# hyperplane-lab/RGBManip

Hardware: AMD Instinct MI355X
Metric: adapose_poses_per_sec_batch256 (higher is better)
Workload: dtype bf16

## Files before the change

### rgbmanip_amd/_lib.py

```python
from __future__ import annotations

import ctypes as C
import os

_HERE = os.path.dirname(os.path.abspath(__file__))
LIB_PATH = os.environ.get("RGBM_HIP_LIB") or os.path.join(_HERE, "librgbm_hip.so")

F32, BF16, F16, BF16X3 = 0, 1, 2, 3
ACT_NONE, ACT_RELU, ACT_PRELU, ACT_TANH = 0, 1, 2, 3
RES_NONE, RES_PRE_ACT, RES_POST_ACT = 0, 1, 2


PROF_ROWS = 42
PROF_KERNELS = [
    ("conv_igemm_glds_kernel<float, 16, 256>", "fp32"), ("conv_igemm_glds_kernel<float, 32, 256>", "fp32"),
    ("conv_igemm_glds_kernel<float, 64, 256>", "fp32"), ("conv_igemm_glds_kernel<float, 128, 128>", "fp32"),
    ("conv_igemm_glds_kernel<unsigned short, 16, 256>", "bf16"), ("conv_igemm_glds_kernel<unsigned short, 32, 256>", "bf16"),
    ("conv_igemm_glds_kernel<unsigned short, 64, 256>", "bf16"), ("conv_igemm_glds_kernel<unsigned short, 128, 128>", "bf16"),
    ("conv3d_tile_kernel<float, ...> (conv1..conv11)", "fp32"), ("conv3d_tile_kernel<unsigned short, ...> (conv1..conv11)", "bf16"),
    ("conv3d_tile_kernel<float, 32, 16, 4, 8, 8, 1, false, true> (conv0 + fused plane sweep)", "fp32"),
    ("conv3d_tile_kernel<unsigned short, 32, 16, 4, 8, 8, 1, false, true> (conv0 + fused plane sweep)", "bf16"),
    ("conv_igemm_ws_kernel<float, ...>", "fp32"), ("conv_igemm_ws_kernel<unsigned short, false, false> (128 channels x 256 pixels)", "bf16"),
    ("conv0_sweep_persistent_kernel<unsigned short> (conv0 + fused plane sweep of bf16 nets; sweep_f16 = 0 / fp16 nets: conv0_sweep_kernel)", "bf16"), ("conv_igemm_ws64_kernel", "bf16"),
    ("conv3d_tile_kernel<unsigned short, 32, 16, 6, 8, 8, 1, false, false> (conv0 on a materialised volume)", "bf16"),
    ("conv3d_tile_kernel<unsigned short, 8, 16, 2, 8, 8, 2, false, false> (conv1)", "bf16"),
    ("conv3d_tile_kernel<unsigned short, 16, 16, 4, 8, 8, 1, false, false> (conv2)", "bf16"),
    ("conv3d_tile_kernel<unsigned short, 16, 32, 2, 8, 8, 2, false, false> (conv3)", "bf16"),
    ("conv3d_tile_kernel<unsigned short, 32, 32, 2, 8, 8, 1, false, false> (conv4)", "bf16"),
    ("conv3d_tile_kernel<unsigned short, 32, 64, 1, 8, 8, 2, false, false> (conv5)", "bf16"),
    ("conv3d_tile_kernel<unsigned short, 64, 64, 1, 8, 8, 1, false, false> (conv6)", "bf16"),
    ("conv3d_tile_kernel<unsigned short, 64, 32, 1, 8, 8, 1, true, false> (conv7)", "bf16"),
    ("conv3d_tile_kernel<unsigned short, 32, 16, 2, 8, 8, 1, true, false> (conv9)", "bf16"),
    ("conv3d_tile_kernel<unsigned short, 16, 16, 4, 8, 8, 1, true, false> (conv11)", "bf16"),
] + [("conv_igemm_glds_kernel<bx3_t, ...> (all channel tiles)", "bf16x3"), ("conv3d_tile_kernel<bx3_t, ...> (conv1..conv11)", "bf16x3"),
     ("conv0 + fused plane sweep <bx3_t>", "bf16x3"), ("conv_igemm_ws_kernel<rgbm::bx3_t, false, false> (128 channels x 256 pixels)", "bf16x3"),
     ("unused (conv_igemm_w256_kernel of rounds 2-5)", "bf16"),
     ("conv_igemm_m32_kernel<unsigned short, 256, 256> (256 channels x 256 pixels, 32x32x16 MFMAs; gemm_kernel = 0: conv_igemm_ws_kernel<unsigned short, true, false>, 256 x 128)", "bf16"),
     ("unused (row-halo ws tile of rounds 2-5)", "bf16"),
     ("conv_igemm_m32_kernel<rgbm::bx3_t, 256, 256> (256 channels x 256 pixels, 32x32x16 MFMAs; gemm_kernel = 0: conv_igemm_ws_kernel<rgbm::bx3_t, true, false>, 256 x 128)", "bf16x3"),
     ("conv_igemm_ws_kernel<rgbm::bx3_t, false, false, true> (64 channels x 256 pixels, four multiply waves)", "bf16x3"),
     ("conv_igemm_ws_kernel<unsigned short, false, false, true> (64 channels x 256 pixels, four multiply waves)", "bf16"),
     ("conv_igemm_ws_kernel<float, false, false, true> (64 channels x 256 pixels, four multiply waves)", "fp32"),
     ("upconv_combine_kernel<16-bit> (PSPUpsample tap combination)", "bf16"), ("upconv_combine_kernel<4-byte> (PSPUpsample tap combination)", "bf16x3"),
     ("upconv_final_kernel (up_3 + final in one kernel; either storage width)", "bf16"),
     ("conv_igemm_m32_kernel<unsigned short, 128, 64 / 128 / 256> (128-pixel tiles: tail and small-batch launches of the 256-channel GEMM)", "bf16"),
     ("conv_igemm_m32_kernel<rgbm::bx3_t, 128, 64 / 128 / 256> (128-pixel tiles: tail and small-batch launches of the 256-channel GEMM)", "bf16x3")]
assert len(PROF_KERNELS) == PROF_ROWS


class RgbmError(RuntimeError):
    pass


class WeightDesc(C.Structure):
    _fields_ = [("name", C.c_char_p), ("data", C.c_void_p), ("ndim", C.c_int), ("shape", C.POINTER(C.c_int64))]


class PolicyLayout(C.Structure):
    _fields_ = [("dims", C.c_int * 5), ("log_std", C.c_int), ("w", (C.c_int * 4) * 2), ("b", (C.c_int * 4) * 2), ("total", C.c_int)]


POLICY_MAX_HIDDEN, POLICY_MAX_WIDTH, POLICY_MAX_ACT = 6, 512, 32
POLICY_ACTIVATIONS = {"elu": 0, "selu": 1, "relu": 2, "crelu": 2, "lrelu": 3, "tanh": 4, "sigmoid": 5}


class PolicyDesc(C.Structure):
    _fields_ = [("obs_dim", C.c_int), ("state_dim", C.c_int), ("act_dim", C.c_int), ("activation", C.c_int), ("asymmetric", C.c_int),
                ("n_hidden", C.c_int * 2), ("hidden", (C.c_int * POLICY_MAX_HIDDEN) * 2),
                ("w", (C.c_int * (POLICY_MAX_HIDDEN + 1)) * 2), ("b", (C.c_int * (POLICY_MAX_HIDDEN + 1)) * 2),
                ("log_std", C.c_int), ("total", C.c_int)]


class AdaposeOut(C.Structure):
    _fields_ = [(n, C.c_void_p) for n in ("view1_nocs", "view2_nocs", "view1_depth", "view2_depth", "view1_r", "view2_r",
                                           "view1_t", "view2_t", "view1_s", "view2_s")]


class ControlRewardArgs(C.Structure):
    _fields_ = [(n, C.c_void_p) for n in ("action", "cam_pose", "target", "move_success", "bbox", "avail", "gt_bbox", "pred_bbox",
                                           "pose_cur", "pose_prev", "robot_pose", "success", "reward", "terms")] + [
        ("coef", C.c_double * 14), ("proper_pos", C.c_double * 3), ("precision2", C.c_double),
        ("N", C.c_int), ("T", C.c_int), ("lda", C.c_int), ("pots", C.c_int), ("first", C.c_int), ("pad_", C.c_int)]


class SynthScene(C.Structure):
    _fields_ = [("cam_pose", C.c_void_p), ("robot_pose", C.c_void_p), ("box", C.c_void_p),
                ("fx", C.c_double), ("fy", C.c_double), ("cx", C.c_double), ("cy", C.c_double),
                ("N", C.c_int), ("H", C.c_int), ("W", C.c_int), ("env0", C.c_int)]


_vp, _i, _f, _d, _sz, _i64 = C.c_void_p, C.c_int, C.c_float, C.c_double, C.c_size_t, C.c_int64
# ... 112 lines not shown
```

### rgbmanip_amd/csrc/adapose.cpp

```cpp
#include "adapose.h"

#include <math.h>
#include <string.h>

namespace rgbm {

static const int kLayerPlanes[4] = {64, 128, 256, 512};
static const int kLayerBlocks[4] = {3, 4, 6, 3};
static const int kLayerStride[4] = {1, 2, 1, 1};
static const int kLayerDil[4] = {1, 1, 2, 4};
static const int kPspBins[4] = {1, 2, 3, 6};
static const int kPspSmallViews = 32;


static const HostTensor* find(const StateDict& sd, const std::string& name) {
  auto it = sd.find(name);
  return it == sd.end() ? nullptr : &it->second;
}

#define GET(var, name)                                               \
  const HostTensor* var = find(sd, name);                            \
  RGBM_REQUIRE(var != nullptr, std::string("missing weight ") + (name))

static int init_conv2d(ConvLayer& L, int dtype, const StateDict& sd, const std::string& wname, const char* bname, int Cin,
// ... 564 lines not shown
  const size_t VP = (size_t)V * P;

  if (int rc = launch_stage_in(P1, P2, choose1, choose2, bf.Pviews, bf.choose, B, P, s)) return rc;
  const float* drop = nullptr;
  if (drop_active()) {
    RGBM_REQUIRE(V <= drop_cap_views && drop_masks && (drop_explicit || drop_state), "dropout: mask buffer smaller than the batch");
    RGBM_REQUIRE((upconv & 3) == 3, "dropout needs option upconv bits 0 and 1 (up_1 / up_2 through the tap combination)");
    if (drop_explicit) {
      RGBM_REQUIRE(drop_explicit == B, "dropout: the masks set for the next forward are for batch " + std::to_string(drop_explicit));
      drop_explicit = 0;
    } else {
      if (int rc = launch_dropout_masks(drop_masks, drop_state, B, drop_p, drop_seed, drop_no_advance ? 0 : 1, s)) return rc;
    }
    drop = drop_masks;
    drop_last_B = B;
  }
  if (int rc = pspnet(bf, V, img1, img2, s, drop)) return rc;
  if (int rc = launch_homography(bf.Pviews, bf.homog, V, B, s)) return rc;
  if (dtype == BF16X3 && !feat_f32_only())
    if (int rc = launch_bx3_to_f32(bf.feat, bf.featf, (long long)V * S * S * 32, s)) return rc;
  if (stop_after == 1) return 0;
  (void)VP; (void)P; (void)D;
  return heads(bf, B, depths, out, s, stop_after);
}

int AdaPose::heads(const Buffers& bf, int B, const float* depths, const Outputs& out, hipStream_t s, int stop_after) const {
  const int V = 2 * B, P = n_pts, S = img, D = n_depth;
  const void* featg = bf.feat;
  int fdt = dtype;
  if (dtype == BF16X3) { featg = bf.featf; fdt = F32; }
  if (feat_f16()) fdt = F16;

  const int Vh = view2_heads ? V : B;
  if (pmlp_table != nullptr && !(g_debug_flags & DBG_POINT_MLP_R5) && ((long long)Vh * P) % 64 == 0) {
    PointMlpDesc pd{};
    pd.table = pmlp_table; pd.feat = featg; pd.choose = bf.choose; pd.nocs4 = bf.nocs4; pd.pf = bf.PF96 + 32; pd.ldpf = 96; pd.P = P; pd.HW = S * S;
    pd.N = (long long)Vh * P;
    if (int rc = launch_point_mlp(fdt, pd, s)) return rc;
  } else {
    if (int rc = launch_gather_points(fdt, featg, bf.choose, bf.X0, Vh, P, S * S, 32, s)) return rc;
    if (int rc = inst.run(bf.X0, bf.X1, Vh, 1, 1, P, 64, nullptr, 0, nullptr, 0, s)) return rc;
    if (int rc = nh[0].run(bf.X1, bf.H128, Vh, 1, 1, P, 128, nullptr, 0, nullptr, 0, s)) return rc;
    if (int rc = nh[1].run(bf.H128, bf.H64, Vh, 1, 1, P, 64, nullptr, 0, nullptr, 0, s)) return rc;
    if (int rc = nh[2].run(bf.H64, bf.nocs4, Vh, 1, 1, P, 4, nullptr, 0, nullptr, 0, s)) return rc;
    if (int rc = npm[0].run(bf.nocs4, bf.N32, Vh, 1, 1, P, 32, nullptr, 0, nullptr, 0, s)) return rc;
    if (int rc = npm[1].run(bf.N32, bf.PF96 + 32, Vh, 1, 1, P, 96, nullptr, 0, nullptr, 0, s)) return rc;
  }

  if (int rc = cost_volume(bf, V, B, depths, s)) return rc;
  if (stop_after == 2) return 0;

  if (int rc = launch_fuse_points(fdt, featg, bf.homog, depths, bf.choose, bf.prob, bf.PF96, V, B, P, D, S, S, 96, 0, s, Vh)) return rc;
  const int pdt = pose_dtype();
  const void* pf_in = bf.PF96;
  if (pdt == F16) {
    if (int rc = launch_f32_to_f16(bf.PF96, bf.PF96h, (long long)Vh * P * 96, s)) return rc;
    pf_in = bf.PF96h;
  } else if (pdt == BF16X3) {
    if (int rc = launch_f32_to_bx3(bf.PF96, bf.PF96, (long long)Vh * P * 96, s)) return rc;
  }
  if (int rc = pm1[0].run(pf_in, bf.Q128a, Vh, 1, 1, P, 128, nullptr, 0, nullptr, 0, s)) return rc;
  if (int rc = pm1[1].run(bf.Q128a, bf.Q128b, Vh, 1, 1, P, 128, nullptr, 0, nullptr, 0, s)) return rc;
  if (int rc = launch_mean_points_partial(pdt, bf.Q128b, (float*)bf.Q128a, Vh, P, 128, s)) return rc;
  if (int rc = launch_view_linear_mean((const float*)bf.Q128a, P, bf.glob, pm2_0_wfull, pm2_0_bias, bf.vbias, Vh, 128, 256, 256, 128, 0, s)) return rc;
  if (int rc = pm2[0].run(bf.Q128b, bf.G256a, Vh, 1, 1, P, 256, nullptr, 0, bf.vbias, 256, s)) return rc;
  if (int rc = pm2[1].run(bf.G256a, bf.G256b, Vh, 1, 1, P, 256, nullptr, 0, nullptr, 0, s)) return rc;
  if (int rc = launch_mean_points_partial(pdt, bf.G256b, (float*)bf.G256a, Vh, P, 256, s)) return rc;
  float* hout[3] = {bf.r6, bf.tv, bf.sv};
  const int hdim[3] = {6, 3, 3};
  if (int rc = launch_pose_heads_mean((const float*)bf.G256a, P, bf.pf2, bf.R, head_w, head_b, hout, hdim, Vh, s)) return rc;

  {
    float* const on[2] = {out.nocs1, out.nocs2};
    float* const od[2] = {out.depth1, out.depth2};
    float* const orr[2] = {out.r1, out.r2};
    float* const ot[2] = {out.t1, out.t2};
    float* const os[2] = {out.s1, out.s2};
    if (int rc = launch_stage_out(bf.nocs4, bf.depth, bf.R, bf.tv, bf.sv, on, od, orr, ot, os, B, P, view2_heads, s)) return rc;
  }
  return 0;
}

int AdaPose::feature_parts(const Buffers& bf, FeaturePart parts[2]) const {
  const size_t one = (size_t)img * img * 32;
  if (dtype != BF16X3) { parts[0] = {bf.feat, 0, one * dtype_size(dtype)}; return 1; }
  if (feat_f32_only()) { parts[0] = {bf.featf, 0, one * 4}; return 1; }
  parts[0] = {bf.feat, 0, one * 4};
  parts[1] = {bf.featf, one * 4, one * 4};
  return 2;
}

size_t AdaPose::feature_bytes() const {
  Buffers bf{};
  FeaturePart parts[2];
  const int n = feature_parts(bf, parts);
  return parts[n - 1].off + parts[n - 1].bytes;
}

size_t AdaPose::features_workspace_bytes(int V) const { return workspace_bytes((V + 1) / 2); }

int AdaPose::features(int V, const float* images, const int* slots, void* pool, int pool_records, void* workspace, size_t workspace_size,
                      hipStream_t s) const {
  RGBM_REQUIRE(V > 0 && pool_records > 0, "features: views and pool records");
  RGBM_REQUIRE(!drop_active(), "features: Dropout2d is on (its masks are drawn per pose and per forward, so a kept feature map would change "
               "what the net computes); the feature cache needs set_dropout(0)");
  RGBM_REQUIRE(((uintptr_t)workspace & 255) == 0 && ((uintptr_t)pool & 15) == 0, "features: workspace must be 256-byte, pool 16-byte aligned");
  const size_t need = features_workspace_bytes(V);
  RGBM_REQUIRE(workspace_size >= need, "features workspace too small: need " + std::to_string(need));
  Arena A(workspace, workspace_size);
  Buffers bf;
  plan((V + 1) / 2, A, bf);
  if (int rc = pspnet(bf, V, images, nullptr, s, nullptr)) return rc;
  if (dtype == BF16X3 && !feat_f32_only())
    if (int rc = launch_bx3_to_f32(bf.feat, bf.featf, (long long)V * img * img * 32, s)) return rc;
  FeaturePart parts[2];
  const int np = feature_parts(bf, parts);
  const size_t rec = feature_bytes();
  for (int i = 0; i < np; ++i)
    if (int rc = launch_feature_store(parts[i].buf, pool, slots, V, pool_records, parts[i].off, parts[i].bytes, rec, s)) return rc;
  return 0;
// ... 31 lines not shown
```

### rgbmanip_amd/csrc/head_kernels.hip

```cpp
#include "common.h"
#include "kernels.h"

namespace rgbm {

template <typename T>
__global__ void gather_points_kernel(const T* __restrict__ feat, const int* __restrict__ choose, float* __restrict__ out,
                                     int V, int P, int HW, int C) {
  const int q = C / 4;
  const long long total = (long long)V * P * q;
  for (long long i = blockIdx.x * (long long)blockDim.x + threadIdx.x; i < total; i += (long long)gridDim.x * blockDim.x) {
    const int c4 = (int)(i % q);
    const long long vp = i / q;
    const long long v = vp / P;
    const int pix = choose[vp];
    float x[4];
    load4(feat + (v * HW + pix) * C + c4 * 4, x);
    store4(out + vp * C + c4 * 4, x);
  }
}

int launch_gather_points(int dtype, const void* feat, const int* choose, float* out, int V, int P, int HW, int C,
                         hipStream_t s) {
  const long long total = (long long)V * P * (C / 4);
  const unsigned g = (unsigned)((total + 255) / 256);
// ... 294 lines not shown
      const bool xin0 = (unsigned)x0 < (unsigned)W, xin1 = (unsigned)(x0 + 1) < (unsigned)W;
      const bool yin0 = (unsigned)y0 < (unsigned)H, yin1 = (unsigned)(y0 + 1) < (unsigned)H;
      const int xc0 = min(max(x0, 0), W - 1), xc1 = min(max(x0 + 1, 0), W - 1);
      const int yc0 = min(max(y0, 0), H - 1), yc1 = min(max(y0 + 1, 0), H - 1);
      float s00[4], s01[4], s10[4], s11[4];
      load4(src + ((long long)yc0 * W + xc0) * C, s00);
      load4(src + ((long long)yc0 * W + xc1) * C, s01);
      load4(src + ((long long)yc1 * W + xc0) * C, s10);
      load4(src + ((long long)yc1 * W + xc1) * C, s11);
      const float w00 = (xin0 && yin0) ? (1.f - tx) * (1.f - ty) : 0.f, w01 = (xin1 && yin0) ? tx * (1.f - ty) : 0.f;
      const float w10 = (xin0 && yin1) ? (1.f - tx) * ty : 0.f, w11 = (xin1 && yin1) ? tx * ty : 0.f;
      const float pr = prob[vp * D + dz];
#pragma unroll
      for (int e = 0; e < 4; ++e) {
        float wv = 0.f;
        if (xin0 && yin0) wv += s00[e] * w00;
        if (xin1 && yin0) wv += s01[e] * w01;
        if (xin0 && yin1) wv += s10[e] * w10;
        if (xin1 && yin1) wv += s11[e] * w11;
        if (!fin) wv = __builtin_nanf("");
        float f = ref[e] + wv;
        if (ROUND_BF16) f = round_through<T>(f);
        acc[e] += f * pr;
      }
    }
    store4(out + vp * ldo + ch_off + c4 * 4, acc);
  }
}

int launch_fuse_points(int dtype, const void* feat, const float* homog, const float* depths, const int* choose,
                       const float* prob, float* out, int V, int B, int P, int D, int H, int W, int ldo, int ch_off,
                       hipStream_t s, int Vn) {
  if (Vn < 0) Vn = V;
  const long long total = (long long)Vn * P * 8;
  RGBM_REQUIRE(D >= 1 && D <= 24 && total > 0 && (total + 255) / 256 < (1ll << 31), "fuse_points supports up to 24 depth planes");
  RGBM_REQUIRE((P & 7) == 0, "fuse_points: the point count must be a multiple of 8 (a wave's 8 points share one view's homography)");
  const unsigned g = (unsigned)((total + 255) / 256);
  if (dtype == BF16)
    hipLaunchKernelGGL((fuse_points_kernel<unsigned short, true>), dim3(g), dim3(256), 0, s, (const unsigned short*)feat,
                       homog, depths, choose, prob, out, V, B, P, D, H, W, ldo, ch_off, Vn);
  else if (dtype == F16)
    hipLaunchKernelGGL((fuse_points_kernel<f16_t, true>), dim3(g), dim3(256), 0, s, (const f16_t*)feat,
                       homog, depths, choose, prob, out, V, B, P, D, H, W, ldo, ch_off, Vn);
  else if (dtype == BF16X3)
    hipLaunchKernelGGL((fuse_points_kernel<bx3_t, false>), dim3(g), dim3(256), 0, s, (const bx3_t*)feat,
                       homog, depths, choose, prob, out, V, B, P, D, H, W, ldo, ch_off, Vn);
  else
    hipLaunchKernelGGL((fuse_points_kernel<float, false>), dim3(g), dim3(256), 0, s, (const float*)feat, homog, depths,
                       choose, prob, out, V, B, P, D, H, W, ldo, ch_off, Vn);
  RGBM_CHECK_HIP(hipGetLastError());
  return 0;
}

constexpr int kMeanSplit = 8;
template <typename TI>
__global__ __launch_bounds__(256) void mean_points_kernel(const TI* __restrict__ in, float* __restrict__ partial, int P, int C) {
  constexpr int E = 16 / sizeof(TI);
  __shared__ float part[256 * E];
  const int v = blockIdx.x / kMeanSplit, sl = blockIdx.x % kMeanSplit;
  const int p0 = (int)((long long)P * sl / kMeanSplit), p1 = (int)((long long)P * (sl + 1) / kMeanSplit);
  const int tpr = C / E, rows = 256 / tpr;
  const int cc = threadIdx.x % tpr, rp = threadIdx.x / tpr;
  float acc[E];
#pragma unroll
  for (int e = 0; e < E; ++e) acc[e] = 0.f;
  if (rp < rows)
#pragma unroll 8
    for (int p = p0 + rp; p < p1; p += rows) {
      float t[E];
      unpack_chunk(*reinterpret_cast<const uint4*>(in + ((long long)v * P + p) * C + cc * E), t, TI());
#pragma unroll
      for (int e = 0; e < E; ++e) acc[e] += t[e];
    }
  if (rp < rows) {
#pragma unroll
    for (int e = 0; e < E; ++e) part[rp * C + cc * E + e] = acc[e];
  }
  __syncthreads();
  for (int c = threadIdx.x; c < C; c += 256) {
    float sum = 0.f;
    for (int r = 0; r < rows; ++r) sum += part[r * C + c];
    partial[(long long)blockIdx.x * C + c] = sum;
  }
}

__device__ __forceinline__ float mean_from_partials(const float* __restrict__ partial, long long v, int c, int C, int P) {
  float sum = 0.f;
#pragma unroll
  for (int sl = 0; sl < kMeanSplit; ++sl) sum += partial[(v * kMeanSplit + sl) * C + c];
  return sum / (float)P;
}

__global__ __launch_bounds__(256) void mean_points_finish_kernel(const float* __restrict__ partial, float* __restrict__ out, int P, int C) {
  const int v = blockIdx.x;
  for (int c = threadIdx.x; c < C; c += 256) out[(long long)v * C + c] = mean_from_partials(partial, v, c, C, P);
}

int launch_mean_points_partial(int dtype, const void* in, float* scratch, int V, int P, int C, hipStream_t s) {
  RGBM_REQUIRE(dtype == F32 || dtype == F16 || dtype == BF16X3, "mean_points: fp32, fp16 or split-pair input");
  RGBM_REQUIRE(scratch != nullptr && (const void*)scratch != in, "mean_points: scratch");
  const int E = dtype == F16 ? 8 : 4;
  RGBM_REQUIRE(C % E == 0 && C / E <= 256 && 256 % (C / E) == 0, "mean_points: channel count");
  const dim3 g((unsigned)V * kMeanSplit);
  if (dtype == F16)
    hipLaunchKernelGGL(mean_points_kernel<f16_t>, g, dim3(256), 0, s, (const f16_t*)in, scratch, P, C);
  else if (dtype == BF16X3)
    hipLaunchKernelGGL(mean_points_kernel<bx3_t>, g, dim3(256), 0, s, (const bx3_t*)in, scratch, P, C);
// ... 251 lines not shown
```

### rgbmanip_amd/csrc/kernels.h

```cpp
#pragma once
#include <vector>

#include "common.h"

namespace rgbm {

int launch_nchw_to_nhwc_pad(int dtype, const float* in, void* out, int V, int C, int H, int W, int Cp, hipStream_t s);
int launch_maxpool3x3s2(int dtype, const void* in, void* out, int V, int H, int W, int C, hipStream_t s);
int launch_resize_bilinear_ac(int dtype, const void* in, void* out, int V, int Hs, int Ws, int C, int Ho, int Wo, int ldo,
                              int ch_off, hipStream_t s);
int launch_copy_channels(int dtype, const void* in, void* out, long long npix, int C, int ldo, int ch_off, hipStream_t s);
int launch_adaptive_avgpool(int dtype, const void* in, void* out, int V, int H, int W, int C, int S, hipStream_t s);
int launch_adaptive_avgpool_multi(int dtype, const void* in, void* const* outs, const int* bins, int nb, int V, int H, int W, int C,
                                  hipStream_t s);
int launch_psp_pool_conv(int dtype, const void* in, int ldi, const void* const* w, void* const* outs, const int* bins, int V, int H, int W,
                         int act, float slope, hipStream_t s);
int launch_psp_resize_cat(int dtype, const void* f, const void* const* stages, const int* bins, void* out, int V, int Ho, int Wo, hipStream_t s);
int launch_homography(const float* P_views, float* out, int V, int B, hipStream_t s);
int launch_build_volume(int dtype, const void* feat, const float* homog, const float* depths, void* vol, int v0, int Vc, int V,
                        int B, int D, int H, int W, hipStream_t s);

int launch_upconv_combine(int dtype, const void* z, const float* bias, void* out, int V, int h, int w, int Co, int ldo, int act,
                          float slope, hipStream_t s, const float* drop = nullptr);
int launch_upconv_final(int dtype, const void* x, const void* wz, const float* bias, float slope, const void* wf, const float* biasf,
                        void* out, int out_f32, int V, int h, int w, hipStream_t s, const void* wf_f16 = nullptr);

constexpr int kDropoutPerView = 256 + 64;
unsigned dropout_threshold(float p);
float dropout_scale(float p);
int launch_dropout_masks(float* masks, unsigned long long* state, int B, float p, unsigned long long seed, int advance, hipStream_t s);

size_t bn_scratch_bytes(int V);
int launch_bn_per_sample(int dtype, void* y, const void* res, const float* gamma, const float* beta, void* scratch, int V,
                         long long nvox, int C, int relu, hipStream_t s);

int launch_to_f32(int dtype, const void* in, float* out, long long n, hipStream_t s);

int launch_gather_points(int dtype, const void* feat, const int* choose, float* out, int V, int P, int HW, int C, hipStream_t s);
int launch_prob_softmax_depth(int dtype, const void* u11, const float* wprob, const int* choose, const float* depths,
                              float* prob, float* depth_out, int v0, int Vc, int B, int P, int D, int H, int W, int classmajor,
                              hipStream_t s);
int launch_fuse_points(int dtype, const void* feat, const float* homog, const float* depths, const int* choose,
                       const float* prob, float* out, int V, int B, int P, int D, int H, int W, int ldo, int ch_off,
                       hipStream_t s, int Vn = -1);
int launch_mean_points(int dtype, const void* in, float* out, float* scratch, int V, int P, int C, hipStream_t s);
int launch_f32_to_f16(const float* in, void* out, long long n, hipStream_t s);
void stem_pack(const float* w, std::vector<float>& packed);
int launch_stem(int dtype, const float* img1, const float* img2, const void* wpk, void* out, int B, int V, int S, hipStream_t s);
int launch_stem_views(int dtype, const float* img, const void* wpk, void* out, int V, int S, hipStream_t s);
int launch_feature_store(const void* src, void* pool, const int* slots, int V, int pool_records, size_t part_off, size_t part_bytes,
                         size_t record_bytes, hipStream_t s);
int launch_feature_gather(const void* pool, void* dst, const int* slot1, const int* slot2, int B, int pool_records, size_t part_off,
                          size_t part_bytes, size_t record_bytes, hipStream_t s);
int launch_feature_bad_slot_nan(const int* slot1, const int* slot2, int B, int pool_records, float* const out[10], const int per_pose[10],
                                hipStream_t s);
int launch_crop_fingerprint(const float* img, int V, int n_words, unsigned long long* keys_out, hipStream_t s);
int launch_f32_to_bx3(const float* in, void* out, long long n, hipStream_t s);
int launch_view_linear(const float* x, const float* W, const float* bias, float* out, int V, int I, int O, int ldw, int i0,
                       int relu, hipStream_t s);
struct PointMlpDesc {
  const float* table;
  const void* feat;
  const int* choose;
  float* nocs4;
  float* pf;
  int ldpf, P, HW;
  long long N;
};
int point_mlp_table_floats();
void point_mlp_pack(const float* const w[6], const float* const b[6], float* table);
int launch_point_mlp(int feat_dtype, const PointMlpDesc& d, hipStream_t s);
int launch_ortho6d(const float* r6, float* R, int V, hipStream_t s);
int launch_mean_points_partial(int dtype, const void* in, float* scratch, int V, int P, int C, hipStream_t s);
int launch_view_linear_mean(const float* partial, int P, float* mean_out, const float* W, const float* bias, float* out, int V, int I, int O,
                            int ldw, int i0, int relu, hipStream_t s);
int launch_pose_heads_mean(const float* partial, int P, float* mean_out, float* R, float* const w[3][3], float* const b[3][3],
                           float* const out[3], const int odim[3], int V, hipStream_t s);
int launch_pose_heads(const float* pf2, float* const w[3][3], float* const b[3][3], float* const out[3], const int odim[3], int V,
                      hipStream_t s);
int launch_stage_in(const float* P1, const float* P2, const int* c1, const int* c2, float* Pviews, int* choose, int B, int P, hipStream_t s);
int launch_stage_out(const float* nocs4, const float* depth, const float* R, const float* tv, const float* sv, float* const nocs[2],
                     float* const dep[2], float* const r[2], float* const t[2], float* const sz[2], int B, int P, int view2, hipStream_t s);
int launch_copy_cols(const float* in, float* out, long long rows, int ldi, int ldo, int n, hipStream_t s);

struct Conv3dTileDesc {
  const void* in; const void* wgt; void* out; const float* bias; const void* res;
  int N, Di, Hi, Wi;
  int Do, Ho, Wo;
  int Dq, Hq, Wq;
  int ntd, nth, ntw;
  int Cout, relu;
  const void* feat; const float* homog; const float* depths; int v0, V, B;
  int prof_variant; double algo_flops, algo_bytes;
  int out_classmajor;
  int feat_f16;
  const int* tile_list; const int* tile_count;
  int tile_mask_stride;
  const unsigned char* tile_mask;
};
enum DebugFlag {
  DBG_NO_WS = 8, DBG_NONUNIFORM_TAPS = 16, DBG_V3_FOR_WS = 64, DBG_NO_WS64 = 128, DBG_NO_ROWHALO = 256, DBG_GENERIC_RESIZE = 512,
  DBG_PSP_STAGE_R5 = 1024, DBG_POINT_MLP_R5 = 2048, DBG_TILE_CONV0 = 4096, DBG_NO_KSPLIT = 16384, DBG_L2_SLIM_TILE = 32768,
  DBG_WS_128x256 = 65536, DBG_NO_SLIM64 = 262144, DBG_KORDER_TAPS_OUTER = 1 << 20, DBG_SWEEP_ALT_BLEND = 1 << 21, DBG_SWEEP_DOT2 = 1 << 22,
  DBG_PP_ONE_KERNEL = 1 << 23, DBG_NO_SLIM_SMALL = 1 << 24, DBG_PP_GENERIC_SELECT = 1 << 25, DBG_PP_GUARD = 1 << 26, DBG_GLOBAL_ADDR = 1 << 27,
  DBG_SWEEP_PER_TILE = 1 << 28, DBG_SPARSE_TAIL_R5 = 1 << 29, DBG_M32_TAILS_R5 = 1 << 30,
};
extern int g_debug_flags;
extern long long g_ws_min_rows;
extern int g_tuning_version;
extern int g_gemm_kernel;
void conv3d_tile_pack(const float* w, const float* scale, int Cin, int Cout, int coutp, bool transposed, int dtype,
                      std::vector<float>& packed);
int launch_conv3d_tile(int layer, int dtype, const Conv3dTileDesc& d, hipStream_t s);
int sparse_mask_bytes_per_view(int S);
int sparse_mask_offset(int S, int layer);
int launch_sparse_masks(const int* choose, int v0, int Vc, int P, int S, unsigned char* masks, int* sweep_list, int* sweep_count,
                        hipStream_t s);
int conv3d_tile_dims(int layer, int dtype, int* TD, int* TH, int* TW);

void conv0_sweep_pack(const float* w, const float* scale, std::vector<float>& packed);
int launch_conv0_sweep(const Conv3dTileDesc& d, int dtype, hipStream_t s);

int conv0_sweep_x3_upload(const std::vector<float>& packed, void** dev);
int launch_conv0_sweep_x3(const Conv3dTileDesc& d, hipStream_t s);
int launch_bx3_to_f32(const void* in, float* out, long long n, hipStream_t s);

int launch_prob_sparse(const void* u9, const void* c0, const void* w11_packed, const float* bias11, const float* wprob,
                       const int* choose, const float* depths, float* prob, float* depth_out, int v0, int Vc, int B, int P,
                       int D, int H, int W, int dtype, hipStream_t s, const void* w11_taps = nullptr);
void prob_sparse_pack(const float* w, const float* scale, std::vector<float>& packed);

int launch_prepare_inputs(const float* rgb, const unsigned char* mask, const double* K, const int* frame_map, int N, int H, int W, int S, int P,
                          unsigned seed, float* img, int* choose, float* pts2d, double* Kcrop, int* window, int* valid,
                          unsigned char* small_scratch, hipStream_t s, int frame0 = 0);

int launch_umeyama_ransac(const float* nocs, const float* depth, const int* choose, const double* Kc, const double* E1,
                          double* bbox, double* srt, int* valid, int B, int P, int img, unsigned seed, hipStream_t s);

int launch_projection(const double* Kc, const double* E, float* P, int n, hipStream_t s);
int launch_pnp_ransac(const float* nocs1, const float* pts1, const float* nocs2, const float* pts2, const double* K, const double* E1,
                      const double* E2, double* bbox, double* srt, int* info, int* valid, int B, int P, unsigned seed, hipStream_t s);

int launch_mask_extent(const unsigned char* mask, int N, int H, int W, int* ext, int* count, hipStream_t s);

int launch_postprocess(const float* nocs, const float* depth, const float* rot, const int* choose, const double* Kc,
                       const double* E1, double* bbox, double* ts_out, int* valid, int B, int P, int img, hipStream_t s,
                       void* scratch = nullptr, size_t scratch_bytes = 0);
int launch_microbench_mfma(float* scratch, int iters, int random_operands, double* flops, hipStream_t s);
int microbench_mfma_scratch_floats(int* n);
int launch_microbench_copy(const void* src, void* dst, size_t bytes, hipStream_t s);
size_t postprocess_scratch_bytes(int B);
int postprocess_slices(int B);

int launch_gae(int T, int N, const float* rewards, const unsigned char* dones, const float* values, const float* last_values,
               float gamma, float lam, float* returns, float* adv, double* sums, hipStream_t s);
int launch_adv_normalise(long long n_local, float* adv, const double* sums, double count_total, hipStream_t s);

struct PolicyLayout { int dims[5]; int log_std; int w[2][4]; int b[2][4]; int total; };
// ... 30 lines not shown
```

Baseline: 5896.

## Fuse pose MLP layers and point sums into two persistent MFMA kernels

Replaces the fp16 pose-MLP path, which was a conversion, four separate 1x1 conv launches and two mean-reduction kernels, with two persistent kernels. Each kernel keeps a 128-point slab's activations in LDS, runs two chained fp16 MFMA layers with bias and ReLU, and accumulates per-slice point sums. The first kernel folds in the fp32-to-fp16 input conversion. The second kernel never writes the 256-channel activations to global memory. This removes launches and intermediate global traffic, at the cost of large LDS per block (one block per CU), a fixed requirement on the point count, and a path that runs only when the pose dtype is F16.

```diff
diff --git a/rgbmanip_amd/_lib.py b/rgbmanip_amd/_lib.py
--- a/rgbmanip_amd/_lib.py
+++ b/rgbmanip_amd/_lib.py
@@ -34,9 +34,9 @@
     ("conv3d_tile_kernel<unsigned short, 16, 16, 4, 8, 8, 1, true, false> (conv11)", "bf16"),
 ] + [("conv_igemm_glds_kernel<bx3_t, ...> (all channel tiles)", "bf16x3"), ("conv3d_tile_kernel<bx3_t, ...> (conv1..conv11)", "bf16x3"),
      ("conv0 + fused plane sweep <bx3_t>", "bf16x3"), ("conv_igemm_ws_kernel<rgbm::bx3_t, false, false> (128 channels x 256 pixels)", "bf16x3"),
-     ("unused (conv_igemm_w256_kernel of rounds 2-5)", "bf16"),
+     ("pose_mlp1_kernel (pose_mlp1.0 + pose_mlp1.2 of a bf16 net in one launch)", "bf16"),
      ("conv_igemm_m32_kernel<unsigned short, 256, 256> (256 channels x 256 pixels, 32x32x16 MFMAs; gemm_kernel = 0: conv_igemm_ws_kernel<unsigned short, true, false>, 256 x 128)", "bf16"),
-     ("unused (row-halo ws tile of rounds 2-5)", "bf16"),
+     ("pose_mlp2_kernel (pose_mlp2.0 + pose_mlp2.2 + the sum over points of a bf16 net in one launch)", "bf16"),
      ("conv_igemm_m32_kernel<rgbm::bx3_t, 256, 256> (256 channels x 256 pixels, 32x32x16 MFMAs; gemm_kernel = 0: conv_igemm_ws_kernel<rgbm::bx3_t, true, false>, 256 x 128)", "bf16x3"),
      ("conv_igemm_ws_kernel<rgbm::bx3_t, false, false, true> (64 channels x 256 pixels, four multiply waves)", "bf16x3"),
      ("conv_igemm_ws_kernel<unsigned short, false, false, true> (64 channels x 256 pixels, four multiply waves)", "bf16"),
diff --git a/rgbmanip_amd/csrc/adapose.cpp b/rgbmanip_amd/csrc/adapose.cpp
--- a/rgbmanip_amd/csrc/adapose.cpp
+++ b/rgbmanip_amd/csrc/adapose.cpp
@@ -640,20 +640,36 @@
 
   if (int rc = launch_fuse_points(fdt, featg, bf.homog, depths, bf.choose, bf.prob, bf.PF96, V, B, P, D, S, S, 96, 0, s, Vh)) return rc;
   const int pdt = pose_dtype();
-  const void* pf_in = bf.PF96;
-  if (pdt == F16) {
-    if (int rc = launch_f32_to_f16(bf.PF96, bf.PF96h, (long long)Vh * P * 96, s)) return rc;
-    pf_in = bf.PF96h;
-  } else if (pdt == BF16X3) {
-    if (int rc = launch_f32_to_bx3(bf.PF96, bf.PF96, (long long)Vh * P * 96, s)) return rc;
-  }
-  if (int rc = pm1[0].run(pf_in, bf.Q128a, Vh, 1, 1, P, 128, nullptr, 0, nullptr, 0, s)) return rc;
-  if (int rc = pm1[1].run(bf.Q128a, bf.Q128b, Vh, 1, 1, P, 128, nullptr, 0, nullptr, 0, s)) return rc;
-  if (int rc = launch_mean_points_partial(pdt, bf.Q128b, (float*)bf.Q128a, Vh, P, 128, s)) return rc;
-  if (int rc = launch_view_linear_mean((const float*)bf.Q128a, P, bf.glob, pm2_0_wfull, pm2_0_bias, bf.vbias, Vh, 128, 256, 256, 128, 0, s)) return rc;
-  if (int rc = pm2[0].run(bf.Q128b, bf.G256a, Vh, 1, 1, P, 256, nullptr, 0, bf.vbias, 256, s)) return rc;
-  if (int rc = pm2[1].run(bf.G256a, bf.G256b, Vh, 1, 1, P, 256, nullptr, 0, nullptr, 0, s)) return rc;
-  if (int rc = launch_mean_points_partial(pdt, bf.G256b, (float*)bf.G256a, Vh, P, 256, s)) return rc;
+  auto pose_layer_ok = [](const ConvLayer& L, int cin, int cout) {
+    return L.dtype == F16 && L.packs.size() == 1 && L.packs[0].ntaps == 1 && L.Cin_pad == cin && L.Cout_pad == cout && L.g.act == ACT_RELU &&
+           L.packs[0].Kpad >= cin && L.bias != nullptr;
+  };
+  const bool pose_fused = pdt == F16 && !(g_debug_flags & DBG_POSE_MLP_R6) && pose_mlp_fits(P) && pose_layer_ok(pm1[0], 96, 128) &&
+                          pose_layer_ok(pm1[1], 128, 128) && pose_layer_ok(pm2[0], 128, 256) && pose_layer_ok(pm2[1], 256, 256);
+  if (pose_fused) {
+    PoseMlpDesc pd{};
+    const ConvLayer* L[4] = {&pm1[0], &pm1[1], &pm2[0], &pm2[1]};
+    for (int l = 0; l < 4; ++l) { pd.w[l] = L[l]->packs[0].w; pd.ldw[l] = L[l]->packs[0].Kpad; pd.bias[l] = L[l]->bias; }
+    pd.pf96 = bf.PF96; pd.vbias = bf.vbias; pd.q128 = bf.Q128b; pd.part128 = (float*)bf.Q128a; pd.part256 = (float*)bf.G256a; pd.V = Vh; pd.P = P;
+    if (int rc = launch_pose_mlp1(pd, s)) return rc;
+    if (int rc = launch_view_linear_mean((const float*)bf.Q128a, P, bf.glob, pm2_0_wfull, pm2_0_bias, bf.vbias, Vh, 128, 256, 256, 128, 0, s)) return rc;
+    if (int rc = launch_pose_mlp2(pd, s)) return rc;
+  } else {
+    const void* pf_in = bf.PF96;
+    if (pdt == F16) {
+      if (int rc = launch_f32_to_f16(bf.PF96, bf.PF96h, (long long)Vh * P * 96, s)) return rc;
+      pf_in = bf.PF96h;
+    } else if (pdt == BF16X3) {
+      if (int rc = launch_f32_to_bx3(bf.PF96, bf.PF96, (long long)Vh * P * 96, s)) return rc;
+    }
+    if (int rc = pm1[0].run(pf_in, bf.Q128a, Vh, 1, 1, P, 128, nullptr, 0, nullptr, 0, s)) return rc;
+    if (int rc = pm1[1].run(bf.Q128a, bf.Q128b, Vh, 1, 1, P, 128, nullptr, 0, nullptr, 0, s)) return rc;
+    if (int rc = launch_mean_points_partial(pdt, bf.Q128b, (float*)bf.Q128a, Vh, P, 128, s)) return rc;
+    if (int rc = launch_view_linear_mean((const float*)bf.Q128a, P, bf.glob, pm2_0_wfull, pm2_0_bias, bf.vbias, Vh, 128, 256, 256, 128, 0, s)) return rc;
+    if (int rc = pm2[0].run(bf.Q128b, bf.G256a, Vh, 1, 1, P, 256, nullptr, 0, bf.vbias, 256, s)) return rc;
+    if (int rc = pm2[1].run(bf.G256a, bf.G256b, Vh, 1, 1, P, 256, nullptr, 0, nullptr, 0, s)) return rc;
+    if (int rc = launch_mean_points_partial(pdt, bf.G256b, (float*)bf.G256a, Vh, P, 256, s)) return rc;
+  }
   float* hout[3] = {bf.r6, bf.tv, bf.sv};
   const int hdim[3] = {6, 3, 3};
   if (int rc = launch_pose_heads_mean((const float*)bf.G256a, P, bf.pf2, bf.R, head_w, head_b, hout, hdim, Vh, s)) return rc;
diff --git a/rgbmanip_amd/csrc/head_kernels.hip b/rgbmanip_amd/csrc/head_kernels.hip
--- a/rgbmanip_amd/csrc/head_kernels.hip
+++ b/rgbmanip_amd/csrc/head_kernels.hip
@@ -370,7 +370,6 @@
   return 0;
 }
 
-constexpr int kMeanSplit = 8;
 template <typename TI>
 __global__ __launch_bounds__(256) void mean_points_kernel(const TI* __restrict__ in, float* __restrict__ partial, int P, int C) {
   constexpr int E = 16 / sizeof(TI);
diff --git a/rgbmanip_amd/csrc/kernels.h b/rgbmanip_amd/csrc/kernels.h
--- a/rgbmanip_amd/csrc/kernels.h
+++ b/rgbmanip_amd/csrc/kernels.h
@@ -76,6 +76,22 @@
                             int ldw, int i0, int relu, hipStream_t s);
 int launch_pose_heads_mean(const float* partial, int P, float* mean_out, float* R, float* const w[3][3], float* const b[3][3],
                            float* const out[3], const int odim[3], int V, hipStream_t s);
+constexpr int kMeanSplit = 8;
+constexpr int kPoseMlpSlab = 128;
+struct PoseMlpDesc {
+  const float* pf96;
+  const void* w[4];
+  int ldw[4];
+  const float* bias[4];
+  const float* vbias;
+  void* q128;
+  float* part128;
+  float* part256;
+  int V, P;
+};
+bool pose_mlp_fits(int P);
+int launch_pose_mlp1(const PoseMlpDesc& d, hipStream_t s);
+int launch_pose_mlp2(const PoseMlpDesc& d, hipStream_t s);
 int launch_pose_heads(const float* pf2, float* const w[3][3], float* const b[3][3], float* const out[3], const int odim[3], int V,
                       hipStream_t s);
 int launch_stage_in(const float* P1, const float* P2, const int* c1, const int* c2, float* Pviews, int* choose, int B, int P, hipStream_t s);
@@ -103,7 +119,7 @@
   DBG_PSP_STAGE_R5 = 1024, DBG_POINT_MLP_R5 = 2048, DBG_TILE_CONV0 = 4096, DBG_NO_KSPLIT = 16384, DBG_L2_SLIM_TILE = 32768,
   DBG_WS_128x256 = 65536, DBG_NO_SLIM64 = 262144, DBG_KORDER_TAPS_OUTER = 1 << 20, DBG_SWEEP_ALT_BLEND = 1 << 21, DBG_SWEEP_DOT2 = 1 << 22,
   DBG_PP_ONE_KERNEL = 1 << 23, DBG_NO_SLIM_SMALL = 1 << 24, DBG_PP_GENERIC_SELECT = 1 << 25, DBG_PP_GUARD = 1 << 26, DBG_GLOBAL_ADDR = 1 << 27,
-  DBG_SWEEP_PER_TILE = 1 << 28, DBG_SPARSE_TAIL_R5 = 1 << 29, DBG_M32_TAILS_R5 = 1 << 30,
+  DBG_SWEEP_PER_TILE = 1 << 28, DBG_SPARSE_TAIL_R5 = 1 << 29, DBG_M32_TAILS_R5 = 1 << 30, DBG_POSE_MLP_R6 = 1 << 19,
 };
 extern int g_debug_flags;
 extern long long g_ws_min_rows;
diff --git a/rgbmanip_amd/csrc/pose_mlp.hip b/rgbmanip_amd/csrc/pose_mlp.hip
--- /dev/null
+++ b/rgbmanip_amd/csrc/pose_mlp.hip
@@ -0,0 +1,323 @@
+#include "common.h"
+#include "kernels.h"
+#include "prof.h"
+
+namespace rgbm {
+
+typedef __attribute__((ext_vector_type(16))) float f32x16;
+
+namespace pose {
+constexpr int SLAB = kPoseMlpSlab;
+constexpr int LD96 = 96 + 8, LD128 = 128 + 8, LD256 = 256 + 8;
+constexpr size_t LDS1 = (size_t)SLAB * (LD96 + 2 * LD128) * sizeof(f16_t);
+constexpr size_t LDS2 = (size_t)SLAB * (LD128 + LD256) * sizeof(f16_t) + 2 * 256 * sizeof(float);
+static_assert(LDS1 <= 160 * 1024 && LDS2 <= 160 * 1024, "pose MLP: a slab's activations must fit the LDS");
+
+__device__ __forceinline__ float relu_sat(float x) {
+  const float r = x < 0.f ? 0.f : x;
+  return r > 65504.f ? 65504.f : r;
+}
+__device__ __forceinline__ f16x4 relu_f16x4(float a, float b, float c, float d) {
+  f16x4 h;
+  h[0] = (f16_t)relu_sat(a); h[1] = (f16_t)relu_sat(b); h[2] = (f16_t)relu_sat(c); h[3] = (f16_t)relu_sat(d);
+  unsigned long long bits = __builtin_bit_cast(unsigned long long, h);
+  asm volatile("" : "+v"(bits));
+  return __builtin_bit_cast(f16x4, bits);
+}
+}
+
+struct PoseMlpArgs {
+  const float* pf96;
+  const f16_t* w[4];
+  int ldw[4];
+  const float* b1; const float* b2; const float* b4;
+  const float* vbias;
+  f16_t* q128;
+  float* part128;
+  float* part256;
+  int P, units;
+};
+
+__global__ __launch_bounds__(512) void pose_mlp1_kernel(const PoseMlpArgs d) {
+  using namespace pose;
+  extern __shared__ __attribute__((aligned(16))) char pose_lds[];
+  f16_t* xs = reinterpret_cast<f16_t*>(pose_lds);
+  f16_t* hs = xs + SLAB * LD96;
+  f16_t* os = hs + SLAB * LD128;
+  const int tid = threadIdx.x, lane = tid & 63, wave = tid >> 6;
+  const int lr = lane & 15, lq = lane >> 4;
+  const int ch0 = wave * 16;
+  if ((int)blockIdx.x >= d.units) return;
+  f16x8 a1[3], a2[4];
+#pragma unroll
+  for (int ks = 0; ks < 3; ++ks) a1[ks] = *reinterpret_cast<const f16x8*>(d.w[0] + (long long)(ch0 + lr) * d.ldw[0] + ks * 32 + lq * 8);
+#pragma unroll
+  for (int ks = 0; ks < 4; ++ks) a2[ks] = *reinterpret_cast<const f16x8*>(d.w[1] + (long long)(ch0 + lr) * d.ldw[1] + ks * 32 + lq * 8);
+  const f32x4 bias1 = *reinterpret_cast<const f32x4*>(d.b1 + ch0 + lq * 4);
+  const f32x4 bias2 = *reinterpret_cast<const f32x4*>(d.b2 + ch0 + lq * 4);
+  const int slice = d.P / kMeanSplit, sps = slice / SLAB;
+
+  auto row0_of = [&](int unit, int sb) { return (long long)(unit / kMeanSplit) * d.P + (long long)(unit % kMeanSplit) * slice + sb * SLAB; };
+  auto load_x = [&](long long row0, float4 (&pre)[6]) {
+#pragma unroll
+    for (int i = 0; i < 6; ++i) {
+      const int idx = tid + 512 * i, r = idx / 24, c4 = idx % 24;
+      pre[i] = *reinterpret_cast<const float4*>(d.pf96 + (row0 + r) * 96 + c4 * 4);
+    }
+  };
+  auto store_x = [&](const float4 (&pre)[6]) {
+#pragma unroll
+    for (int i = 0; i < 6; ++i) {
+      const int idx = tid + 512 * i, r = idx / 24, c4 = idx % 24;
+      f16x4 h;
+      h[0] = (f16_t)sat_f16(pre[i].x); h[1] = (f16_t)sat_f16(pre[i].y); h[2] = (f16_t)sat_f16(pre[i].z); h[3] = (f16_t)sat_f16(pre[i].w);
+      *reinterpret_cast<f16x4*>(xs + r * LD96 + c4 * 4) = h;
+    }
+  };
+
+  int unit = blockIdx.x, sb = 0;
+  float4 pre[6];
+  load_x(row0_of(unit, sb), pre);
+  store_x(pre);
+  float sum[4] = {0.f, 0.f, 0.f, 0.f};
+  while (true) {
+    const long long row0 = row0_of(unit, sb);
+    __syncthreads();
+    {
+      f32x4 acc[8];
+#pragma unroll
+      for (int t = 0; t < 8; ++t) acc[t] = f32x4{0.f, 0.f, 0.f, 0.f};
+#pragma unroll
+      for (int ks = 0; ks < 3; ++ks)
+#pragma unroll
+        for (int t = 0; t < 8; ++t) {
+          const f16x8 b = *reinterpret_cast<const f16x8*>(xs + (t * 16 + lr) * LD96 + ks * 32 + lq * 8);
+          acc[t] = __builtin_amdgcn_mfma_f32_16x16x32_f16(a1[ks], b, acc[t], 0, 0, 0);
+        }
+#pragma unroll
+      for (int t = 0; t < 8; ++t)
+        *reinterpret_cast<f16x4*>(hs + (t * 16 + lr) * LD128 + ch0 + lq * 4) =
+            relu_f16x4(acc[t][0] + bias1[0], acc[t][1] + bias1[1], acc[t][2] + bias1[2], acc[t][3] + bias1[3]);
+    }
+    __syncthreads();
+    int nunit = unit, nsb = sb + 1;
+    if (nsb == sps) { nsb = 0; nunit += gridDim.x; }
+    const bool has_next = nunit < d.units;
+    if (has_next) load_x(row0_of(nunit, nsb), pre);
+    {
+      f32x4 acc[8];
+#pragma unroll
+      for (int t = 0; t < 8; ++t) acc[t] = f32x4{0.f, 0.f, 0.f, 0.f};
+#pragma unroll
+      for (int ks = 0; ks < 4; ++ks)
+#pragma unroll
+        for (int t = 0; t < 8; ++t) {
+          const f16x8 b = *reinterpret_cast<const f16x8*>(hs + (t * 16 + lr) * LD128 + ks * 32 + lq * 8);
+          acc[t] = __builtin_amdgcn_mfma_f32_16x16x32_f16(a2[ks], b, acc[t], 0, 0, 0);
+        }
+#pragma unroll
+      for (int t = 0; t < 8; ++t) {
+        const f16x4 h = relu_f16x4(acc[t][0] + bias2[0], acc[t][1] + bias2[1], acc[t][2] + bias2[2], acc[t][3] + bias2[3]);
+        *reinterpret_cast<f16x4*>(os + (t * 16 + lr) * LD128 + ch0 + lq * 4) = h;
+#pragma unroll
+        for (int i = 0; i < 4; ++i) sum[i] += (float)h[i];
+      }
+    }
+    if (has_next) store_x(pre);
+    __syncthreads();
+#pragma unroll
+    for (int i = 0; i < 4; ++i) {
+      const int idx = tid + 512 * i, r = idx >> 4, c = idx & 15;
+      *reinterpret_cast<uint4*>(d.q128 + (row0 + r) * 128 + c * 8) = *reinterpret_cast<const uint4*>(os + r * LD128 + c * 8);
+    }
+    if (nsb == 0) {
+#pragma unroll
+      for (int i = 0; i < 4; ++i) {
+        float s = sum[i];
+        s += __shfl_xor(s, 1); s += __shfl_xor(s, 2); s += __shfl_xor(s, 4); s += __shfl_xor(s, 8);
+        sum[i] = s;
+      }
+      if (lr == 0) *reinterpret_cast<float4*>(d.part128 + (long long)unit * 128 + ch0 + lq * 4) = make_float4(sum[0], sum[1], sum[2], sum[3]);
+#pragma unroll
+      for (int i = 0; i < 4; ++i) sum[i] = 0.f;
+    }
+    if (!has_next) break;
+    unit = nunit; sb = nsb;
+  }
+}
+
+__global__ __launch_bounds__(512) void pose_mlp2_kernel(const PoseMlpArgs d) {
+  using namespace pose;
+  extern __shared__ __attribute__((aligned(16))) char pose_lds[];
+  f16_t* xs = reinterpret_cast<f16_t*>(pose_lds);
+  f16_t* hs = xs + SLAB * LD128;
+  float* vb = reinterpret_cast<float*>(hs + SLAB * LD256);
+  float* b4 = vb + 256;
+  const int tid = threadIdx.x, lane = tid & 63, wave = tid >> 6;
+  const int lr = lane & 31, lh = lane >> 5;
+  const int ch0 = wave * 32;
+  if ((int)blockIdx.x >= d.units) return;
+  f16x8 a3[8], a4[16];
+  auto load_a3 = [&]() {
+    const f16_t* p = d.w[2] + (long long)(ch0 + lr) * d.ldw[2] + lh * 8;
+    asm volatile("" : "+v"(p));
+#pragma unroll
+    for (int ks = 0; ks < 8; ++ks) a3[ks] = *reinterpret_cast<const f16x8*>(p + ks * 16);
+  };
+  load_a3();
+#pragma unroll
+  for (int ks = 0; ks < 16; ++ks) a4[ks] = *reinterpret_cast<const f16x8*>(d.w[3] + (long long)(ch0 + lr) * d.ldw[3] + ks * 16 + lh * 8);
+  if (tid < 256) b4[tid] = d.b4[tid];
+  const int slice = d.P / kMeanSplit, sps = slice / SLAB;
+
+  auto row0_of = [&](int unit, int sb) { return (long long)(unit / kMeanSplit) * d.P + (long long)(unit % kMeanSplit) * slice + sb * SLAB; };
+  const int xr = tid >> 4, xc = (tid & 15) * 8;
+  f32x4 pre0, pre1, pre2, pre3;
+  auto load_x = [&](long long row0) {
+    const f16_t* p = d.q128 + (row0 + xr) * 128 + xc;
+    pre0 = *reinterpret_cast<const f32x4*>(p);
+    pre1 = *reinterpret_cast<const f32x4*>(p + 32 * 128);
+    pre2 = *reinterpret_cast<const f32x4*>(p + 64 * 128);
+    pre3 = *reinterpret_cast<const f32x4*>(p + 96 * 128);
+  };
+  auto store_x = [&]() {
+    f16_t* p = xs + xr * LD128 + xc;
+    *reinterpret_cast<f32x4*>(p) = pre0;
+    *reinterpret_cast<f32x4*>(p + 32 * LD128) = pre1;
+    *reinterpret_cast<f32x4*>(p + 64 * LD128) = pre2;
+    *reinterpret_cast<f32x4*>(p + 96 * LD128) = pre3;
+  };
+
+  int unit = blockIdx.x, sb = 0;
+  load_x(row0_of(unit, sb));
+  store_x();
+  float sum[16];
+#pragma unroll
+  for (int i = 0; i < 16; ++i) sum[i] = 0.f;
+  while (true) {
+    if (sb == 0 && tid < 256) vb[tid] = d.vbias[(long long)(unit / kMeanSplit) * 256 + tid];
+    __syncthreads();
+#pragma unroll
+    for (int tp = 0; tp < 2; ++tp) {
+      f32x16 acc[2];
+#pragma unroll
+      for (int u = 0; u < 2; ++u)
+#pragma unroll
+        for (int i = 0; i < 16; ++i) acc[u][i] = 0.f;
+#pragma unroll
+      for (int ks = 0; ks < 8; ++ks)
+#pragma unroll
+        for (int u = 0; u < 2; ++u) {
+          const f16x8 b = *reinterpret_cast<const f16x8*>(xs + ((tp * 2 + u) * 32 + lr) * LD128 + ks * 16 + lh * 8);
+          acc[u] = __builtin_amdgcn_mfma_f32_32x32x16_f16(a3[ks], b, acc[u], 0, 0, 0);
+        }
+#pragma unroll
+      for (int u = 0; u < 2; ++u)
+#pragma unroll
+        for (int g = 0; g < 4; ++g) {
+          const int c = ch0 + 8 * g + 4 * lh;
+          const f32x4 bv = *reinterpret_cast<const f32x4*>(vb + c);
+          *reinterpret_cast<f16x4*>(hs + ((tp * 2 + u) * 32 + lr) * LD256 + c) =
+              relu_f16x4(acc[u][4 * g] + bv[0], acc[u][4 * g + 1] + bv[1], acc[u][4 * g + 2] + bv[2], acc[u][4 * g + 3] + bv[3]);
+          __builtin_amdgcn_sched_barrier(0);
+        }
+    }
+    __syncthreads();
+    int nunit = unit, nsb = sb + 1;
+    if (nsb == sps) { nsb = 0; nunit += gridDim.x; }
+    const bool has_next = nunit < d.units;
+    if (has_next) load_x(row0_of(nunit, nsb));
+#pragma unroll
+    for (int tp = 0; tp < 2; ++tp) {
+      f32x16 acc[2];
+#pragma unroll
+      for (int u = 0; u < 2; ++u)
+#pragma unroll
+        for (int i = 0; i < 16; ++i) acc[u][i] = 0.f;
+#pragma unroll
+      for (int ks = 0; ks < 16; ++ks)
+#pragma unroll
+        for (int u = 0; u < 2; ++u) {
+          const f16x8 b = *reinterpret_cast<const f16x8*>(hs + ((tp * 2 + u) * 32 + lr) * LD256 + ks * 16 + lh * 8);
+          acc[u] = __builtin_amdgcn_mfma_f32_32x32x16_f16(a4[ks], b, acc[u], 0, 0, 0);
+        }
+#pragma unroll
+      for (int u = 0; u < 2; ++u)
+#pragma unroll
+        for (int g = 0; g < 4; ++g) {
+          const f32x4 bv = *reinterpret_cast<const f32x4*>(b4 + ch0 + 8 * g + 4 * lh);
+          const f16x4 h = relu_f16x4(acc[u][4 * g] + bv[0], acc[u][4 * g + 1] + bv[1], acc[u][4 * g + 2] + bv[2], acc[u][4 * g + 3] + bv[3]);
+#pragma unroll
+          for (int i = 0; i < 4; ++i) sum[4 * g + i] += (float)h[i];
+          __builtin_amdgcn_sched_barrier(0);
+        }
+    }
+    if (has_next) { load_a3(); store_x(); }
+    if (nsb == 0) {
+#pragma unroll
+      for (int i = 0; i < 16; ++i) {
+        float s = sum[i];
+        s += __shfl_xor(s, 1); s += __shfl_xor(s, 2); s += __shfl_xor(s, 4); s += __shfl_xor(s, 8); s += __shfl_xor(s, 16);
+        sum[i] = s;
+      }
+      if (lr == 0) {
+#pragma unroll
+        for (int g = 0; g < 4; ++g)
+          *reinterpret_cast<float4*>(d.part256 + (long long)unit * 256 + ch0 + 8 * g + 4 * lh) =
+              make_float4(sum[4 * g], sum[4 * g + 1], sum[4 * g + 2], sum[4 * g + 3]);
+      }
+#pragma unroll
+      for (int i = 0; i < 16; ++i) sum[i] = 0.f;
+    }
+    if (!has_next) break;
+    unit = nunit; sb = nsb;
+  }
+}
+
+bool pose_mlp_fits(int P) { return P > 0 && P % (kMeanSplit * kPoseMlpSlab) == 0; }
+
+static int pose_mlp_args(const PoseMlpDesc& d, PoseMlpArgs& a) {
+  RGBM_REQUIRE(d.V > 0 && pose_mlp_fits(d.P), "pose MLP: points per view must be a multiple of 8 slabs of 128");
+  RGBM_REQUIRE(d.pf96 && d.q128 && d.part128 && d.part256 && d.vbias && d.bias[0] && d.bias[1] && d.bias[3], "pose MLP: buffers");
+  const int K[4] = {96, 128, 128, 256};
+  for (int l = 0; l < 4; ++l) {
+    RGBM_REQUIRE(d.w[l] != nullptr && d.ldw[l] >= K[l] && d.ldw[l] % 8 == 0 && ((uintptr_t)d.w[l] & 15) == 0, "pose MLP: weight rows of 16-byte chunks");
+    a.w[l] = reinterpret_cast<const f16_t*>(d.w[l]);
+    a.ldw[l] = d.ldw[l];
+  }
+  RGBM_REQUIRE((long long)d.V * kMeanSplit < (1ll << 31), "pose MLP: views");
+  a.pf96 = d.pf96; a.b1 = d.bias[0]; a.b2 = d.bias[1]; a.b4 = d.bias[3]; a.vbias = d.vbias;
+  a.q128 = reinterpret_cast<f16_t*>(d.q128); a.part128 = d.part128; a.part256 = d.part256;
+  a.P = d.P; a.units = d.V * kMeanSplit;
+  return 0;
+}
+
+int launch_pose_mlp1(const PoseMlpDesc& d, hipStream_t s) {
+  PoseMlpArgs a;
+  if (int rc = pose_mlp_args(d, a)) return rc;
+  int n_cu = 0;
+  if (int rc = persistent_grid_cus(&n_cu)) return rc;
+  if (int rc = ensure_dynamic_lds(reinterpret_cast<const void*>(pose_mlp1_kernel), (int)pose::LDS1)) return rc;
+  const double n = (double)d.V * d.P;
+  prof_begin_launch(s, 30, 2.0 * n * (96.0 * 128 + 128.0 * 128), n * (96 * 4 + 128 * 2) + (double)a.units * 128 * 4);
+  hipLaunchKernelGGL(pose_mlp1_kernel, dim3(a.units < n_cu ? a.units : n_cu), dim3(512), pose::LDS1, s, a);
+  prof_end_launch(s);
+  RGBM_CHECK_HIP(hipGetLastError());
+  return 0;
+}
+
+int launch_pose_mlp2(const PoseMlpDesc& d, hipStream_t s) {
+  PoseMlpArgs a;
+  if (int rc = pose_mlp_args(d, a)) return rc;
+  int n_cu = 0;
+  if (int rc = persistent_grid_cus(&n_cu)) return rc;
+  if (int rc = ensure_dynamic_lds(reinterpret_cast<const void*>(pose_mlp2_kernel), (int)pose::LDS2)) return rc;
+  const double n = (double)d.V * d.P;
+  prof_begin_launch(s, 32, 2.0 * n * (128.0 * 256 + 256.0 * 256), n * 128 * 2 + (double)a.units * 256 * 4);
+  hipLaunchKernelGGL(pose_mlp2_kernel, dim3(a.units < n_cu ? a.units : n_cu), dim3(512), pose::LDS2, s, a);
+  prof_end_launch(s);
+  RGBM_CHECK_HIP(hipGetLastError());
+  return 0;
+}
+
+}
```

Result: faster. 5969, median of 6 (+1.2%).
